# secondmind-labs/trieste

Hardware: NVIDIA H100
Metric: acquisition candidate-points/sec (EI on GPR N=4096 fp64) (higher is better)
Workload: dtype f64

## Files before the change

trieste_b200/csrc/kernels_f64.cuh:

```cuda
#pragma once
#include "common.cuh"
#include "../../include/trieste_b200.h"
#include "kernel_fn.cuh"
#include <cfloat>

namespace tb {

template <int KIND, int DP>
__global__ void __launch_bounds__(512)
kstar_panels_kernel(const double* __restrict__ Xs,
                    const double* __restrict__ alpha,
                    const double* __restrict__ Xc,
                    const double* __restrict__ inv_ls,
                    int N, int nkc, int D, int64_t M, int64_t cand0, double variance,
                    double mean_const, double* __restrict__ KsP, double* __restrict__ mean_out) {
  const int lane = threadIdx.x & 31, tj = threadIdx.x >> 5;
  const int tl = lane >> 2, kq = lane & 3;
  const int t_local = tj * 8 + tl;
  const int64_t t = cand0 + (int64_t)blockIdx.x * BT + t_local;
  const bool valid = t < M;

  double xc[DP];
#pragma unroll
  for (int d = 0; d < DP; ++d) xc[d] = (valid && d < D) ? Xc[t * D + d] * inv_ls[d] : 0.0;
// ... 379 lines not shown
}
__device__ __forceinline__ double gibbon_repulsion_value(double var, double noise, double uu, double w) {
  const double yvar = var + noise;
  return w * (0.5 * (log(yvar - uu) - log(yvar)));
}
__device__ __forceinline__ double gibbon_value(int acq, const double* __restrict__ samp, int ns, double mean, double var,
                                               double noise, double uu, double w) {
  if (acq == TB_ACQ_GIBBON_QUALITY) return gibbon_quality_value(samp, ns, mean, var, noise);
  const double rep = gibbon_repulsion_value(var, noise, uu, w);
  if (acq == TB_ACQ_GIBBON_REPULSION) return rep;
  return rep + gibbon_quality_value(samp, ns, mean, var, noise);
}

__device__ __forceinline__ void penalty_factor(int kind, double dist, double radius, double scale, double& f, double& w) {
  if (kind == TB_PEN_SOFT) {
    const double z = (dist - radius) / scale;
    f = ndtr_tfp(z);
    double lc, ratio;
    mes_terms(-z, lc, ratio);
    w = dist > 0.0 ? ratio / (scale * dist) : 0.0;
  } else {
    const double u = dist / (radius + scale);
    f = pow(pow(u, -5.0) + 1.0, -0.2);
    const double u5 = u * u * u * u * u;
    w = dist > 0.0 ? (1.0 / dist) / (dist * (1.0 + u5)) : 0.0;
  }
}

constexpr int PEN_TILE = 32;
constexpr int PEN_DMAX = 32;

struct TailPenalty {
  const double* xc = nullptr;
  const double* pend = nullptr;
  const double* radius = nullptr;
  const double* scale = nullptr;
  double* grad = nullptr;
  int P = 0, D = 0, kind = 0;
  const double* gib_uu = nullptr;
  double gib_w = 0.0;
};

__device__ __forceinline__ void block_best_store(double bv, int64_t bi, double* __restrict__ blk_best, int64_t* __restrict__ blk_idx) {
#pragma unroll
  for (int o = 16; o > 0; o >>= 1) {
    double v2 = __shfl_xor_sync(0xffffffffu, bv, o);
    int64_t i2 = __shfl_xor_sync(0xffffffffu, bi, o);
    best_merge(bv, bi, v2, i2);
  }
  __shared__ double sv[8];
  __shared__ int64_t si[8];
  if ((threadIdx.x & 31) == 0) {
    sv[threadIdx.x >> 5] = bv;
    si[threadIdx.x >> 5] = bi;
  }
  __syncthreads();
  if (threadIdx.x == 0) {
    for (int w = 1; w < (int)(blockDim.x >> 5); ++w) best_merge(bv, bi, sv[w], si[w]);
    blk_best[blockIdx.x] = bv;
    blk_idx[blockIdx.x] = bi;
  }
}

__device__ __forceinline__ double chunk_raw_variance(const double* __restrict__ partial, int G, int64_t McPad, int64_t t,
                                                     double variance) {
  double ss = 0.0;
  for (int g = 0; g < G; ++g) ss += partial[(int64_t)g * McPad + t];
  return variance - ss;
}

template <bool PEN>
__global__ void __launch_bounds__(256)
tail_kernel(const double* __restrict__ partial, int G, int64_t McPad, const double* __restrict__ mean,
            int64_t Mc, int64_t idx0, double variance, int acq, double param, double aux,
            const double* __restrict__ samp, int nsamp, double* __restrict__ out_vals, double* __restrict__ out_mean, double* __restrict__ out_var,
            double* __restrict__ blk_best, int64_t* __restrict__ blk_idx, const int64_t* __restrict__ idx_map, const TailPenalty pen) {
  const int64_t t = (int64_t)blockIdx.x * blockDim.x + threadIdx.x;
  double bv = -INFINITY;
  int64_t bi = INT64_MAX;
  double vb = 0.0;
  if (t < Mc) {
    double var = fmax(chunk_raw_variance(partial, G, McPad, t, variance), 1e-12);
    double mu = mean[t];
    if (out_mean) out_mean[t] = mu;
    if (out_var) out_var[t] = var;
    if (acq >= 0) {
      double v = (acq == TB_ACQ_MES) ? mes_value(samp, nsamp, mu, var)
                 : (acq >= TB_ACQ_GIBBON_QUALITY)
                     ? gibbon_value(acq, samp, nsamp, mu, var, aux, pen.gib_uu ? pen.gib_uu[t] : 0.0, pen.gib_w)
                     : acq_value(acq, param, aux, mu, var);
      if (PEN) {
        vb = v;
      } else {
        if (out_vals) out_vals[t] = v;
        if (v == v) { bv = v; bi = idx_map ? idx_map[t] : idx0 + t; }
      }
    }
  }
  if (PEN) {
    __shared__ double sp[PEN_TILE * PEN_DMAX], sr[PEN_TILE], sc[PEN_TILE];
    const bool live = t < Mc && acq >= 0;
    const int D = pen.D;
    double x[PEN_DMAX], g[PEN_DMAX];
#pragma unroll
    for (int d = 0; d < PEN_DMAX; ++d) {
      x[d] = (live && d < D) ? pen.xc[t * D + d] : 0.0;
      g[d] = 0.0;
    }
    double prod = 1.0;
    for (int j0 = 0; j0 < pen.P; j0 += PEN_TILE) {
      const int nj = min(PEN_TILE, pen.P - j0);
      __syncthreads();
      for (int i = threadIdx.x; i < nj * D; i += blockDim.x) sp[i] = pen.pend[(int64_t)j0 * D + i];
      if (threadIdx.x < nj) {
        sr[threadIdx.x] = pen.radius[j0 + threadIdx.x];
        sc[threadIdx.x] = pen.scale[j0 + threadIdx.x];
      }
      __syncthreads();
      if (!live) continue;
      for (int j = 0; j < nj; ++j) {
        double r2 = 0.0;
#pragma unroll
        for (int d = 0; d < PEN_DMAX; ++d)
          if (d < D) {
            const double df = x[d] - sp[j * D + d];
            r2 = fma(df, df, r2);
          }
        double f, w;
        penalty_factor(pen.kind, sqrt(r2), sr[j], sc[j], f, w);
        prod *= f;
        if (pen.grad) {
#pragma unroll
          for (int d = 0; d < PEN_DMAX; ++d)
            if (d < D) g[d] = fma(w, x[d] - sp[j * D + d], g[d]);
        }
      }
    }
    if (live) {
      const double v = vb < 0.0 ? NAN : vb * prod;
      if (pen.grad) {
        double* gr = pen.grad + t * D;
#pragma unroll
        for (int d = 0; d < PEN_DMAX; ++d)
          if (d < D) gr[d] = fma(prod, gr[d], prod == 0.0 ? 0.0 : vb * (prod * g[d]));
      }
      if (out_vals) out_vals[t] = v;
      if (v == v) { bv = v; bi = idx_map ? idx_map[t] : idx0 + t; }
    }
  }
  if (blk_best == nullptr) return;
  block_best_store(bv, bi, blk_best, blk_idx);
}

__global__ void __launch_bounds__(256)
argmax_fold_kernel(const double* __restrict__ blk_best, const int64_t* __restrict__ blk_idx, int nblk,
                   double* __restrict__ run_best, int64_t* __restrict__ run_idx) {
  double bv = -INFINITY;
  int64_t bi = INT64_MAX;
  for (int i = threadIdx.x; i < nblk; i += blockDim.x) best_merge(bv, bi, blk_best[i], blk_idx[i]);
#pragma unroll
  for (int o = 16; o > 0; o >>= 1) {
    double v2 = __shfl_xor_sync(0xffffffffu, bv, o);
    int64_t i2 = __shfl_xor_sync(0xffffffffu, bi, o);
    best_merge(bv, bi, v2, i2);
  }
  __shared__ double sv[8];
  __shared__ int64_t si[8];
  if ((threadIdx.x & 31) == 0) {
    sv[threadIdx.x >> 5] = bv;
    si[threadIdx.x >> 5] = bi;
  }
  __syncthreads();
  if (threadIdx.x == 0) {
    for (int w = 1; w < 8; ++w) best_merge(bv, bi, sv[w], si[w]);
    double rv = *run_best;
    int64_t ri = *run_idx;
    best_merge(rv, ri, bv, bi);
    *run_best = rv;
    *run_idx = ri;
  }
}

__device__ __forceinline__ double screen_threshold(int acq, double tau, double var_ub) {
  const double m = acq == TB_ACQ_EI ? fma(0x1p-20, fabs(tau), 0x1p-36 * sqrt(var_ub)) : 0x1p-20 * fmax(1.0, fabs(tau));
  return tau - m;
}

}
```

trieste_b200/csrc/prescreen.cuh:

```cuda
#pragma once
#include <cuda_fp16.h>
#include "kernels_f64.cuh"

namespace tb {
namespace pre {

constexpr int KS = 64;
constexpr int KH = 32;
constexpr int TH = 256;
template <int DP> struct Cpt { static constexpr int value = DP <= 12 ? 4 : DP <= 20 ? 2 : 1; };
template <int DP> struct Row { static constexpr int W = ((DP + 3 + 3) / 4) * 4; };

__host__ __device__ constexpr int tc_nk(int dp) { return (3 * dp + 2 + 15) / 16; }
__host__ __device__ constexpr int tc_mt(int dp) { return tc_nk(dp) <= 2 ? 4 : tc_nk(dp) <= 4 ? 2 : 1; }
__host__ __device__ constexpr int tc_slices(int dp) { return tc_nk(dp) <= 2 ? 16 : 8; }
__host__ __device__ constexpr int tc_slice_bytes(int dp) { return 256 * tc_nk(dp) + 32; }
__host__ __device__ constexpr int tc_cands(int dp) { return 16 * tc_mt(dp) * (TH / 32); }

struct Bound {
  double rel;
  double lin;
  double lin_max;
  double abs;
  double safety;
// ... 143 lines not shown
  asm("mma.sync.aligned.m16n8k16.row.col.f32.f16.f16.f32 {%0,%1,%2,%3}, {%4,%5,%6,%7}, {%8,%9}, {%0,%1,%2,%3};"
      : "+f"(c[0]), "+f"(c[1]), "+f"(c[2]), "+f"(c[3])
      : "r"(a[0]), "r"(a[1]), "r"(a[2]), "r"(a[3]), "r"(b0), "r"(b1));
}

template <int KIND, int DP>
__global__ void __launch_bounds__(TH, 2)
tc_mean_bounds_kernel(const unsigned char* __restrict__ cols, int nsl, int npos_sl, const double* __restrict__ Xc,
                      const double* __restrict__ inv_ls, const double* __restrict__ centre, int D, int64_t M,
                      const __grid_constant__ Bound b, int acq, double param, double var_ub, double* __restrict__ out0,
                      double* __restrict__ out1, double* __restrict__ blk_best, int64_t* __restrict__ blk_idx) {
  constexpr int NK = tc_nk(DP), K = 16 * NK, MT = tc_mt(DP), SL = tc_slices(DP), SLB = tc_slice_bytes(DP);
  constexpr int CB = tc_cands(DP), STB = SL * SLB;
  constexpr int CAND_BYTES = CB * (2 * K + 4), SMEM = CAND_BYTES > 2 * STB ? CAND_BYTES : 2 * STB;
  static_assert(KIND != TB_MATERN12 && STB % 16 == 0 && SMEM <= 48 * 1024, "tc_mean_bounds_kernel geometry");
  __shared__ __align__(16) unsigned char sm[SMEM];
  const int64_t c0 = (int64_t)blockIdx.x * CB;
  {
    __half* sa = reinterpret_cast<__half*>(sm);
    float* sx2 = reinterpret_cast<float*>(sm + CB * 2 * K);
    for (int c = threadIdx.x; c < CB; c += TH) {
      const int64_t t = c0 + c;
      __half* row = sa + c * K;
      float x2 = 0.0f;
#pragma unroll
      for (int d = 0; d < DP; ++d) {
        const float x = (t < M && d < D) ? (float)((Xc[t * D + d] * inv_ls[d] - centre[d]) * b.pre) : 0.0f;
        x2 = fmaf(x, x, x2);
        const __half hi = __float2half_rn(x);
        row[d] = row[2 * DP + d] = hi;
        row[DP + d] = __float2half_rn(x - __half2float(hi));
      }
      row[3 * DP] = row[3 * DP + 1] = __float2half_rn(1.0f);
#pragma unroll
      for (int k = 3 * DP + 2; k < K; ++k) row[k] = __float2half_rn(0.0f);
      sx2[c] = x2;
    }
  }
  __syncthreads();
  const int warp = threadIdx.x >> 5, lane = threadIdx.x & 31, g = lane >> 2, tg = lane & 3;
  uint32_t af[MT][NK][4];
  float cx[MT][2];
#pragma unroll
  for (int m = 0; m < MT; ++m) {
    const int r = (warp * MT + m) * 16 + g;
    const __half* sa = reinterpret_cast<const __half*>(sm);
#pragma unroll
    for (int kk = 0; kk < NK; ++kk) {
      const __half* p = sa + r * K + kk * 16 + 2 * tg;
      af[m][kk][0] = *reinterpret_cast<const uint32_t*>(p);
      af[m][kk][1] = *reinterpret_cast<const uint32_t*>(p + 8 * K);
      af[m][kk][2] = *reinterpret_cast<const uint32_t*>(p + 8);
      af[m][kk][3] = *reinterpret_cast<const uint32_t*>(p + 8 * K + 8);
    }
    const float* sx2 = reinterpret_cast<const float*>(sm + CB * 2 * K);
    cx[m][0] = sx2[r];
    cx[m][1] = sx2[r + 8];
  }
  __syncthreads();

  auto stage_load = [&](int kc, int buf) {
    const unsigned char* src = cols + (int64_t)kc * STB;
#pragma unroll
    for (int i = 0; i < (STB / 16 + TH - 1) / TH; ++i) {
      const int e = i * TH + (int)threadIdx.x;
      if (e < STB / 16) asm volatile("cp.async.cg.shared.global [%0], [%1], 16;" ::"r"(smem_u32(sm + buf * STB + 16 * e)), "l"(src + 16 * e) : "memory");
    }
    asm volatile("cp.async.commit_group;" ::: "memory");
  };
  auto slice = [&](const unsigned char* sp, float (&acc)[MT][2]) {
    uint32_t bf[NK][2];
    if constexpr (NK % 2 == 0) {
#pragma unroll
      for (int kk = 0; kk < NK; kk += 2) {
        const uint4 v = reinterpret_cast<const uint4*>(sp)[(lane * NK + kk) / 2];
        bf[kk][0] = v.x, bf[kk][1] = v.y, bf[kk + 1][0] = v.z, bf[kk + 1][1] = v.w;
      }
    } else {
#pragma unroll
      for (int kk = 0; kk < NK; ++kk) {
        const uint2 v = reinterpret_cast<const uint2*>(sp)[lane * NK + kk];
        bf[kk][0] = v.x, bf[kk][1] = v.y;
      }
    }
    const float2 w = reinterpret_cast<const float2*>(sp + 256 * NK)[tg];
#pragma unroll
    for (int m = 0; m < MT; ++m) {
      float c[4] = {cx[m][0], cx[m][0], cx[m][1], cx[m][1]};
#pragma unroll
      for (int kk = 0; kk < NK; ++kk) mma_f16(c, af[m][kk], bf[kk][0], bf[kk][1]);
#pragma unroll
      for (int i = 0; i < 4; ++i) {
        acc[m][i >> 1] = fmaf(i & 1 ? w.y : w.x, kfun<KIND>(c[i]), acc[m][i >> 1]);
      }
    }
  };

  double pd[MT][2], qd[MT][2];
#pragma unroll
  for (int m = 0; m < MT; ++m) pd[m][0] = pd[m][1] = qd[m][0] = qd[m][1] = 0.0;
  const int nst = (nsl + SL - 1) / SL;
  stage_load(0, 0);
  for (int kc = 0; kc < nst; ++kc) {
    const int buf = kc & 1;
    if (kc + 1 < nst) {
      stage_load(kc + 1, buf ^ 1);
      asm volatile("cp.async.wait_group 1;" ::: "memory");
    } else {
      asm volatile("cp.async.wait_group 0;" ::: "memory");
    }
    __syncthreads();
    const unsigned char* st = sm + buf * STB;
    const int s0 = kc * SL, pe = min(SL, nsl - s0), bnd = min(max(npos_sl - s0, 0), pe);
    auto run = [&](int sa, int sb, double (&dd)[MT][2]) {
      float acc[MT][2];
#pragma unroll
      for (int m = 0; m < MT; ++m) acc[m][0] = acc[m][1] = 0.0f;
#pragma unroll 1
      for (int s = sa; s < sb; ++s) slice(st + s * SLB, acc);
#pragma unroll
      for (int m = 0; m < MT; ++m) dd[m][0] += (double)acc[m][0], dd[m][1] += (double)acc[m][1];
    };
    run(0, bnd, pd);
    run(bnd, pe, qd);
    __syncthreads();
  }
  double bv = -INFINITY;
  int64_t bi = INT64_MAX;
#pragma unroll
  for (int m = 0; m < MT; ++m)
#pragma unroll
    for (int h = 0; h < 2; ++h) {
      pd[m][h] += __shfl_xor_sync(0xffffffffu, pd[m][h], 1);
      qd[m][h] += __shfl_xor_sync(0xffffffffu, qd[m][h], 1);
      pd[m][h] += __shfl_xor_sync(0xffffffffu, pd[m][h], 2);
      qd[m][h] += __shfl_xor_sync(0xffffffffu, qd[m][h], 2);
      const int64_t t = c0 + (warp * MT + m) * 16 + g + 8 * h;
      if ((2 * m + h) % 4 != tg || t >= M) continue;
      const double x2 = (double)cx[m][h];
      const double lg = x2 < 0x1p28 ? b.lin * (x2 + b.x2max) : NAN;
      bound_out(b, t, lg, pd[m][h] - qd[m][h], pd[m][h] + qd[m][h], acq, param, var_ub, out0, out1, bv, bi);
    }
  if (acq >= 0) block_best_store(bv, bi, blk_best, blk_idx);
}

__global__ void probe_kernel(const double* __restrict__ Xc, int D, const int64_t* __restrict__ probe, double* __restrict__ xsel,
                             int64_t* __restrict__ isel) {
  int64_t p = *probe;
  if (p == INT64_MAX) p = 0;
  for (int d = threadIdx.x; d < D; d += blockDim.x) xsel[d] = Xc[p * D + d];
  if (threadIdx.x == 0) isel[0] = p;
}

__global__ void __launch_bounds__(256)
compact_kernel(const double* __restrict__ Xc, const double* __restrict__ ub, int64_t M, int64_t split, int D, double var_ub,
               int acq, const double* __restrict__ run_best, int64_t cap, unsigned long long* __restrict__ count,
               double* __restrict__ xsel, int64_t* __restrict__ isel) {
  const int64_t t = (int64_t)blockIdx.x * blockDim.x + threadIdx.x;
  const double thr = screen_threshold(acq, *run_best, var_ub);
  const bool keep = t < M && !(ub[t] < thr);
  const bool back = t >= split;
  const unsigned ball = __ballot_sync(0xffffffffu, keep);
  if (ball == 0u) return;
  const int lane = threadIdx.x & 31;
  const unsigned bb = __ballot_sync(0xffffffffu, keep && back), bf = ball & ~bb;
  unsigned long long base_f = 0, base_b = 0;
  if (lane == 0) {
    if (bf) base_f = atomicAdd(&count[0], (unsigned long long)__popc(bf));
    if (bb) base_b = atomicAdd(&count[1], (unsigned long long)__popc(bb));
  }
  base_f = __shfl_sync(0xffffffffu, base_f, 0);
  base_b = __shfl_sync(0xffffffffu, base_b, 0);
  if (!keep) return;
  const unsigned below = (1u << lane) - 1u;
  const int64_t r = back ? (int64_t)(base_b + (unsigned long long)__popc(bb & below)) : (int64_t)(base_f + (unsigned long long)__popc(bf & below));
  if (r >= cap) return;
  const int64_t pos = back ? cap - 1 - r : r;
  for (int d = 0; d < D; ++d) xsel[pos * D + d] = Xc[t * D + d];
  isel[pos] = t;
}

}
}
```

trieste_b200/csrc/tb_api.cu:

```cuda
#include "gp_handle.cuh"
#include "kernels_extra.cuh"
#include "prescreen.cuh"
#include "batch_ei.cuh"
#include "ehvi.cuh"
#include "int8_engines.h"
#include <chrono>
#include "factor.cuh"
#include "lbfgs.cuh"

using namespace tb;
namespace tb {
int kernels_init();
}

namespace tb {

__global__ void scale_inputs_kernel(const double* __restrict__ X, const double* __restrict__ inv_ls,
                                    int64_t N, int D, int DP, int64_t rows, double* __restrict__ Xs) {
  int64_t i = (int64_t)blockIdx.x * blockDim.x + threadIdx.x;
  if (i >= rows * DP) return;
  int64_t k = i / DP;
  int d = (int)(i % DP);
  Xs[i] = (k < N && d < D) ? X[k * D + d] * inv_ls[d] : 0.0;
}
// ... 978 lines not shown
                         + 4.01 * std::ldexp(1.0, -22)
                         + 1.01 * rd * std::ldexp(1.0, -25)
                         + pre::tc_nk(DP) * 2.01 * 24 * std::ldexp(1.0, -23);
    const double abs_q = 1.01 * rd * std::ldexp(1.0, -24) + std::ldexp(1.0, -25);
    const double lin_tc = cq * lin_q + l64;
    bool f16_ok = false;
    if (1.01 * lin_tc * (box2 + 1.01 * x2max) <= 0.5 * lin_max) {
      tc = prescreen_tc_columns(h, N, DP, W, &gp->pre_nsl, &gp->pre_npos_sl, &f16_ok);
      gp->pre_tc = f16_ok;
    }
    if (gp->pre_tc) {
      terms = 8.0 * gp->pre_nsl;
      lin = lin_tc;
      rel += cq * abs_q;
    }
  } else {
    lin = LN2 * u;
  }
  gp->pre_rel = 1.01 * rel;
  gp->pre_lin = 1.01 * lin;
  gp->pre_lin_max = lin_max;
  gp->pre_abs = 1.01 * (asum * (2700.0 * std::ldexp(1.0, -126) + kappa * tail) + 2.0 * terms * std::ldexp(1.0, -149));
  gp->pre_scale = pre;
  gp->pre_x2max = 1.01 * x2max;
  const size_t bytes = gp->pre_tc ? tc.size() : sizeof(float) * h.size();
  TB_TRY(gp->dPreRows.reserve(bytes));
  TB_TRY(gp->dPreCentre.reserve(sizeof(double) * DP));
  TB_CUDA(cudaMemcpyAsync(gp->dPreRows.p, gp->pre_tc ? (const void*)tc.data() : (const void*)h.data(), bytes, cudaMemcpyHostToDevice, st));
  TB_CUDA(cudaMemcpyAsync(gp->dPreCentre.p, centre.data(), sizeof(double) * DP, cudaMemcpyHostToDevice, st));
  TB_CUDA(cudaStreamSynchronize(st));
  gp->pre_gen = gp->cache_gen;
  return 0;
}

static int prescreen_blocks(const tb_gp* gp, int64_t M) {
  const int DP = gp->DP;
  const int64_t per = gp->pre_tc ? pre::tc_cands(DP) : (int64_t)pre::TH * (DP <= 12 ? 4 : DP <= 20 ? 2 : 1);
  return (int)((M + per - 1) / per);
}

static int launch_mean_bounds(tb_gp* gp, cudaStream_t st, const double* Xc, int64_t M, int acq, double param, double var_ub,
                              double* out0, double* out1, double* blk_best, int64_t* blk_idx) {
  TB_TRY(prescreen_ensure(gp));
  pre::Bound b;
  b.rel = gp->pre_rel;
  b.lin = gp->pre_lin;
  b.lin_max = gp->pre_lin_max;
  b.abs = gp->pre_abs;
  b.safety = 4.0;
  b.x2max = gp->pre_x2max;
  b.mean_const = gp->mean_const;
  b.pre = gp->pre_scale;
  const int D = gp->D;
  const double* il = gp->dInvLs.as<double>();
  const double* cen = gp->dPreCentre.as<double>();
  const unsigned blocks = (unsigned)prescreen_blocks(gp, M);
  with_kind_dp(gp->kernel, gp->DP, [&](auto K, auto P) {
    constexpr int KIND = decltype(K)::value, DP = decltype(P)::value;
    if (!gp->pre_tc) {
      const int nst = (int)((gp->N + pre::KS - 1) / pre::KS);
      pre::mean_bounds_kernel<KIND, DP><<<blocks, pre::TH, 0, st>>>(gp->dPreRows.as<float>(), nst, Xc, il, cen, D, M, b, acq, param,
                                                                    var_ub, out0, out1, blk_best, blk_idx);
    } else if constexpr (KIND != TB_MATERN12) {
      pre::tc_mean_bounds_kernel<KIND, DP><<<blocks, pre::TH, 0, st>>>(gp->dPreRows.as<unsigned char>(), gp->pre_nsl, gp->pre_npos_sl,
                                                                       Xc, il, cen, D, M, b, acq, param, var_ub, out0, out1, blk_best,
                                                                       blk_idx);
    }
  });
  TB_LAUNCHED();
  TB_CUDA(cudaGetLastError());
  return 0;
}

enum class Engine {
  F64,
  OZ21,
  OZ15,
};

static int select_engine(tb_gp* gp, bool need_v, Engine* eng) {
  if (!(gp->engine == 1 && gp->N <= 16384)) {
    if (need_v) TB_TRY(ensure_upper_panels(gp));
    *eng = Engine::F64;
    return 0;
  }
  if (need_v) TB_TRY(ensure_kinv_dense(gp));
  bool single_pass;
  TB_TRY(int8_select(gp, need_v, &single_pass));
  *eng = single_pass ? Engine::OZ15 : Engine::OZ21;
  return 0;
}

static int eng_tile_width(const tb_gp* gp, Engine e) { return e == Engine::F64 ? BT : int8_tile_width(gp, e == Engine::OZ15); }
static size_t eng_tile_bytes(const tb_gp* gp, Engine e) {
  return e == Engine::F64 ? (size_t)gp->nkc * PANEL * sizeof(double) : int8_tile_bytes(gp, e == Engine::OZ15);
}

static int eng_groups(const tb_gp* gp, Engine e, int tiles) {
  const int fill = (2 * NUM_SMS + tiles - 1) / tiles;
  if (e == Engine::F64) return tiles >= NUM_SMS ? 1 : std::max(1, std::min(fill, gp->NB));
  return std::max(std::max(1, (gp->NB + 3) / 4), std::min(gp->NB, fill));
}

static int eng_kstar(tb_gp* gp, Engine e, const double* xc, int64_t mc, int tiles, const KSplit* split = nullptr, bool wide = false) {
  double* mean = gp->sMean.as<double>();
  if (e == Engine::F64) return launch_kstar(gp, xc, mc, tiles, gp->sKs.as<double>(), mean);
  return int8_kstar(gp, e == Engine::OZ15, xc, mc, tiles, gp->sKs.as<int8_t>(), mean, split, wide);
}

static int eng_variance(tb_gp* gp, Engine e, int tiles, int G, int64_t McPad, bool packed_a, int kper = 0) {
  cudaStream_t st = gp->stream;
  double* partial = gp->sPartial.as<double>();
  if (e != Engine::F64) return int8_variance(gp, e == Engine::OZ15, gp->sKs.as<int8_t>(), tiles, G, McPad, partial, kper);
  if (packed_a)
    trigemm_kernel<false, EPI_SUMSQ_PACKED><<<dim3(tiles, G), TG_THREADS, TG_SMEM, st>>>(
        gp->dLinvP.as<double>(), gp->sKs.as<double>(), gp->NB, gp->nkc, G, McPad, partial, gp->sA.as<double>(), nullptr, 0);
  else
    trigemm_kernel<false, EPI_SUMSQ><<<dim3(tiles, G), TG_THREADS, TG_SMEM, st>>>(
        gp->dLinvP.as<double>(), gp->sKs.as<double>(), gp->NB, gp->nkc, G, McPad, partial, nullptr, nullptr, 0);
  TB_LAUNCHED();
  TB_CUDA(cudaGetLastError());
  return 0;
}

static int eng_store_a(tb_gp* gp, Engine e, int tiles, int64_t McPad, double* out) {
  const int64_t lda = (int64_t)gp->NB * BM;
  const int G = eng_groups(gp, e, tiles);
  if (e != Engine::F64) return int8_store(gp, e == Engine::OZ15, false, gp->sKs.as<int8_t>(), tiles, G, McPad, out, lda);
  trigemm_kernel<false, EPI_PLAIN><<<dim3(tiles, G), TG_THREADS, TG_SMEM, gp->stream>>>(gp->dLinvP.as<double>(), gp->sKs.as<double>(),
                                                                                        gp->NB, gp->nkc, G, McPad, nullptr, nullptr, out, lda);
  TB_LAUNCHED();
  TB_CUDA(cudaGetLastError());
  return 0;
}

static int eng_store_v(tb_gp* gp, Engine e, int tiles, int64_t McPad) {
  const int64_t ldv = (int64_t)gp->NB * BM;
  double* V = gp->sV.as<double>();
  if (e == Engine::OZ21) {
    const int G = std::max(1, std::min(gp->NB, std::max((gp->NB + 7) / 8, (2 * NUM_SMS + tiles - 1) / tiles)));
    return int8_store(gp, false, true, gp->sKs.as<int8_t>(), tiles, G, McPad, V, ldv);
  }
  const int G = eng_groups(gp, e, tiles);
  if (e == Engine::OZ15) return int8_store(gp, true, true, gp->sKs.as<int8_t>(), tiles, G, McPad, V, ldv);
  trigemm_kernel<true, EPI_PLAIN><<<dim3(tiles, G), TG_THREADS, TG_SMEM, gp->stream>>>(gp->dLinvTP.as<double>(), gp->sA.as<double>(), gp->NB,
                                                                                       gp->NB * (BM / BK), G, McPad, nullptr, nullptr, V, ldv);
  TB_LAUNCHED();
  TB_CUDA(cudaGetLastError());
  return 0;
}


static int argmax_reset(tb_gp* gp) {
  const double init_v = -INFINITY;
  const int64_t init_i = INT64_MAX;
  TB_CUDA(cudaMemcpyAsync(gp->sRun.p, &init_v, 8, cudaMemcpyHostToDevice, gp->stream));
  TB_CUDA(cudaMemcpyAsync((char*)gp->sRun.p + 8, &init_i, 8, cudaMemcpyHostToDevice, gp->stream));
  return 0;
}
static int argmax_begin(tb_gp* gp, int64_t chunk_cap) {
  const int tail_blocks_cap = (int)((chunk_cap + 255) / 256);
  TB_TRY(gp->sRun.reserve(16));
  TB_TRY(gp->sBlkBest.reserve(sizeof(double) * tail_blocks_cap));
  TB_TRY(gp->sBlkIdx.reserve(sizeof(int64_t) * tail_blocks_cap));
  return argmax_reset(gp);
}
static int argmax_fold(tb_gp* gp, int64_t n) {
  argmax_fold_kernel<<<1, 256, 0, gp->stream>>>(gp->sBlkBest.as<double>(), gp->sBlkIdx.as<int64_t>(), (int)((n + 255) / 256),
                                                gp->sRun.as<double>(), reinterpret_cast<int64_t*>((char*)gp->sRun.p + 8));
  TB_LAUNCHED();
  return 0;
}
static int argmax_end(tb_gp* gp, EvalRequest& rq) {
  TB_CUDA(cudaMemcpyAsync(&rq.best_value, gp->sRun.p, 8, cudaMemcpyDeviceToHost, gp->stream));
  TB_CUDA(cudaMemcpyAsync(&rq.best_index, (char*)gp->sRun.p + 8, 8, cudaMemcpyDeviceToHost, gp->stream));
  return 0;
}

template <class F>
static int profiled_gemm(tb_gp* gp, double flops, F&& launch) {
  if (!gp->profile) return launch();
  cudaEvent_t e0 = nullptr, e1 = nullptr;
  TB_CUDA(cudaEventCreate(&e0));
  TB_CUDA(cudaEventCreate(&e1));
  TB_CUDA(cudaEventRecord(e0, gp->stream));
  TB_TRY(launch());
  TB_CUDA(cudaEventRecord(e1, gp->stream));
  gp->prof_events.emplace_back(e0, e1);
  gp->prof_event_flops.push_back(flops);
  return 0;
}
static int profile_fold(tb_gp* gp) {
  for (size_t i = 0; i < gp->prof_events.size(); ++i) {
    float ms = 0.f;
    TB_CUDA(cudaEventElapsedTime(&ms, gp->prof_events[i].first, gp->prof_events[i].second));
    gp->prof_ms += ms;
    gp->prof_flops += gp->prof_event_flops[i];
    gp->prof_launches += 1;
    cudaEventDestroy(gp->prof_events[i].first);
    cudaEventDestroy(gp->prof_events[i].second);
  }
  gp->prof_events.clear();
  gp->prof_event_flops.clear();
  return 0;
}

struct EvalOut {
  double *vals = nullptr, *mean = nullptr, *var = nullptr, *grad = nullptr;
};

static int member_step(tb_gp* gp, Engine e, const double* xc, int64_t n, int Gfix, bool grad, int* G, int64_t* McPad,
                       const KSplit* split = nullptr, bool spread = false) {
  const int nt = eng_tile_width(gp, e);
  const int tiles = (int)((n + nt - 1) / nt);
  *G = Gfix ? Gfix : eng_groups(gp, e, tiles);
  *McPad = (int64_t)tiles * nt;
  const int kper = spread && e != Engine::F64 ? int8_split_kper(gp, e == Engine::OZ15, tiles, *G) : 0;
  TB_TRY(eng_kstar(gp, e, xc, n, tiles, split, kper > 0));
  TB_TRY(profiled_gemm(gp, (double)*McPad * (double)gp->N * (double)gp->N,
                       [&] { return eng_variance(gp, e, tiles, *G, *McPad, grad, kper); }));
  return grad ? eng_store_v(gp, e, tiles, *McPad) : 0;
}

static int eval_chunk(tb_gp* gp, const EvalRequest& rq, Engine e, const double* xc, int64_t n, int64_t c0, int Gfix, const EvalOut& o,
                      const int64_t* idx_map = nullptr, const KSplit* split = nullptr) {
  cudaStream_t st = gp->stream;
  const double* partial = gp->sPartial.as<double>();
  const double* mean = gp->sMean.as<double>();
  int G;
  int64_t McPad;
  TB_TRY(member_step(gp, e, xc, n, Gfix, o.grad != nullptr, &G, &McPad, split, idx_map != nullptr));
  if (o.grad) {
    TB_TRY(launch_partials(gp, st, rq.acq, rq.param, partial, G, McPad, mean, xc, n));
    TB_TRY(launch_grad(gp, xc, n, o.grad));
  }
  TB_TRY(launch_tail(gp, st, rq, partial, G, McPad, mean, n, c0, o.vals, o.mean, o.var, xc, o.grad, idx_map));
  return rq.want_argmax ? argmax_fold(gp, n) : 0;
}

static int argmax_screened(tb_gp* gp, const EvalRequest& rq, Engine e, int64_t chunk_cap, int G, bool* done) {
  *done = false;
  cudaStream_t st = gp->stream;
  const int D = gp->D, nt = eng_tile_width(gp, e);
  const int64_t M = rq.M;
  const int64_t cap = std::max<int64_t>(1, M / 4);
  TB_TRY(prescreen_ensure(gp));
  const int sblocks = (int)((M + 255) / 256), bblocks = prescreen_blocks(gp, M);
  TB_TRY(gp->sScrUb.reserve(sizeof(double) * (size_t)M));
  TB_TRY(gp->sScrX.reserve(sizeof(double) * (size_t)cap * D));
  TB_TRY(gp->sScrIdx.reserve(sizeof(int64_t) * (size_t)cap));
  TB_TRY(gp->sScrBlk.reserve(16 * (size_t)bblocks + 32));
  double* ub = gp->sScrUb.as<double>();
  double* xsel = gp->sScrX.as<double>();
  int64_t* isel = gp->sScrIdx.as<int64_t>();
  double* bb = gp->sScrBlk.as<double>();
  int64_t* bi = reinterpret_cast<int64_t*>(bb + bblocks);
  double* probe_v = reinterpret_cast<double*>(bi + bblocks);
  int64_t* probe_i = reinterpret_cast<int64_t*>(probe_v + 1);
  unsigned long long* count = reinterpret_cast<unsigned long long*>(probe_v + 2);
  const int64_t split = ((M - 1) / chunk_cap) * chunk_cap;
  const KSplit ks_full = int8_kstar_split(gp, e == Engine::OZ15, (int)(chunk_cap / nt)),
               ks_last = int8_kstar_split(gp, e == Engine::OZ15, (int)((M - split + nt - 1) / nt));
  const bool same_split = ks_full.ksplit == ks_last.ksplit && ks_full.kc_per == ks_last.kc_per;
  const double var_ub = std::fmax(gp->variance, 1e-12);
  const double init_v = -INFINITY;
  const int64_t init_i = INT64_MAX;
  TB_CUDA(cudaMemcpyAsync(probe_v, &init_v, 8, cudaMemcpyHostToDevice, st));
  TB_CUDA(cudaMemcpyAsync(probe_i, &init_i, 8, cudaMemcpyHostToDevice, st));
  TB_TRY(launch_mean_bounds(gp, st, rq.Xc, M, rq.acq, rq.param, var_ub, ub, nullptr, bb, bi));
  argmax_fold_kernel<<<1, 256, 0, st>>>(bb, bi, bblocks, probe_v, probe_i);
  TB_LAUNCHED();
  pre::probe_kernel<<<1, 32, 0, st>>>(rq.Xc, D, probe_i, xsel, isel);
  TB_LAUNCHED();
  bool probe_last = true;
  if (!same_split) {
    int64_t p = 0;
    TB_CUDA(cudaMemcpyAsync(&p, probe_i, 8, cudaMemcpyDeviceToHost, st));
    TB_CUDA(cudaStreamSynchronize(st));
    probe_last = (p == INT64_MAX ? 0 : p) >= split;
  }
  const EvalOut none;
  TB_TRY(eval_chunk(gp, rq, e, xsel, 1, 0, G, none, isel, probe_last ? &ks_last : &ks_full));
  TB_CUDA(cudaMemsetAsync(count, 0, 16, st));
  pre::compact_kernel<<<sblocks, 256, 0, st>>>(rq.Xc, ub, M, split, D, var_ub, rq.acq, gp->sRun.as<double>(), cap, count, xsel, isel);
  TB_LAUNCHED();
  unsigned long long n[2] = {0, 0};
  TB_CUDA(cudaMemcpyAsync(n, count, 16, cudaMemcpyDeviceToHost, st));
  TB_CUDA(cudaStreamSynchronize(st));
  TB_CUDA(cudaGetLastError());
  if (n[0] + n[1] > (unsigned long long)cap) return argmax_reset(gp);
  const int64_t nf = (int64_t)n[0], nb = (int64_t)n[1];
  for (int64_t s0 = 0; s0 < nf; s0 += chunk_cap)
    TB_TRY(eval_chunk(gp, rq, e, xsel + s0 * D, std::min<int64_t>(chunk_cap, nf - s0), 0, G, none, isel + s0, &ks_full));
  for (int64_t s0 = cap - nb; s0 < cap; s0 += chunk_cap)
    TB_TRY(eval_chunk(gp, rq, e, xsel + s0 * D, std::min<int64_t>(chunk_cap, cap - s0), 0, G, none, isel + s0, &ks_last));
  *done = true;
  return 0;
}

struct ChunkPlan {
  int64_t chunk_cap = 0;
  int G[EHVI_LMAX] = {};
};
static ChunkPlan plan_chunks(tb_gp* const* gps, const Engine* eng, int n, bool grad, int64_t M) {
  ChunkPlan p;
  const size_t budget = (size_t)1280 << 20;
  for (int l = 0; l < n; ++l) {
    const tb_gp* gp = gps[l];
    const Engine e = eng[l];
    const int nt = eng_tile_width(gp, e);
    int64_t max_tiles;
    if (e != Engine::F64 && !grad) {
      max_tiles = std::max<int64_t>(1, (int64_t)(budget / eng_tile_bytes(gp, e)));
      if (max_tiles >= 2 * NUM_SMS) max_tiles = (max_tiles / (2 * NUM_SMS)) * (2 * NUM_SMS);
      else if (max_tiles >= NUM_SMS) max_tiles = NUM_SMS;
      max_tiles = std::min<int64_t>(max_tiles, 8 * NUM_SMS);
    } else if (e == Engine::OZ15) {
      const size_t v_bytes = (size_t)nt * gp->NB * BM * sizeof(double);
      max_tiles = std::max<int64_t>(1, (int64_t)(budget / std::max(eng_tile_bytes(gp, e), v_bytes)));
      if (max_tiles >= NUM_SMS) max_tiles = (max_tiles / NUM_SMS) * NUM_SMS;
    } else {
      max_tiles = chunk_tiles(gp);
    }
    const int64_t cap = std::min<int64_t>(max_tiles * nt, ((M + nt - 1) / nt) * nt);
    p.chunk_cap = l == 0 ? cap : std::min(p.chunk_cap, cap);
  }
  for (int l = 0; l < n; ++l) {
    const int nt = eng_tile_width(gps[l], eng[l]);
    if (eng[l] != Engine::F64 && !grad) p.G[l] = eng_groups(gps[l], eng[l], (int)((p.chunk_cap + nt - 1) / nt));
  }
  return p;
}

static int reserve_chunk(tb_gp* gp, Engine e, bool grad, int64_t chunk_cap, int G) {
  const int nt = eng_tile_width(gp, e);
  const int64_t tiles_cap = (chunk_cap + nt - 1) / nt, pad_cap = tiles_cap * nt;
  TB_TRY(gp->sKs.reserve((size_t)tiles_cap * eng_tile_bytes(gp, e)));
  TB_TRY(gp->sPartial.reserve(sizeof(double) * (size_t)(G ? G : gp->NB) * pad_cap));
  TB_TRY(gp->sMean.reserve(sizeof(double) * pad_cap));
  if (grad) {
    if (e == Engine::F64) TB_TRY(gp->sA.reserve((size_t)tiles_cap * gp->NB * (BM / BK) * PANEL * sizeof(double)));
    TB_TRY(gp->sV.reserve((size_t)pad_cap * gp->NB * BM * sizeof(double)));
    TB_TRY(gp->sMisc.reserve(sizeof(double) * 2 * pad_cap));
  }
  return 0;
}

static int check_eval(const tb_gp* gp, const EvalRequest& rq) {
  TB_CHECK(gp->cache_valid, "posterior cache is not built: call tb_gp_update_posterior_cache first");
  TB_CHECK(rq.M >= 0, "negative candidate count");
  if (rq.want_argmax) TB_CHECK(rq.M > 0, "argmax over an empty candidate set");
  return 0;
}

static int run_eval(tb_gp* gp, EvalRequest& rq) {
  TB_CUDA(cudaSetDevice(gp->device));
  cudaStream_t st = gp->stream;
  const int D = gp->D;
  const bool grad = rq.out_grad != nullptr;
  if (rq.M == 0) return 0;
  if (grad) TB_CHECK(rq.acq >= 0, "gradients need an acquisition kind");
  Engine e;
  TB_TRY(select_engine(gp, grad, &e));
  const ChunkPlan cp = plan_chunks(&gp, &e, 1, grad, rq.M);
  const int64_t chunk_cap = cp.chunk_cap;
  const Staged<const double> xin(rq.Xc, D, gp->sXc, st);
  const Staged<double> vals(rq.out_vals, 1, gp->sVals, st), mean(rq.out_mean, 1, gp->sMean, st), var(rq.out_var, 1, gp->sVar, st),
      grads(rq.out_grad, D, gp->sGrad, st);
  TB_TRY(reserve_chunk(gp, e, grad, chunk_cap, cp.G[0]));
  TB_TRY(xin.reserve(chunk_cap));
  TB_TRY(vals.reserve(chunk_cap));
  TB_TRY(var.reserve(chunk_cap));
  TB_TRY(grads.reserve(chunk_cap));
  if (rq.want_argmax) TB_TRY(argmax_begin(gp, chunk_cap));

  bool screened = false;
  if (e != Engine::F64 && argmax_screen_wanted(rq, xin.dev)) TB_TRY(argmax_screened(gp, rq, e, chunk_cap, cp.G[0], &screened));
  const int64_t m_loop = screened ? 0 : rq.M;
  for (int64_t c0 = 0; c0 < m_loop; c0 += chunk_cap) {
    const int64_t mc = std::min<int64_t>(chunk_cap, rq.M - c0);
    const double* xc;
    TB_TRY(xin.in(c0, mc, &xc));
    EvalOut o;
    o.vals = vals.out(c0);
    o.mean = mean.host() ? nullptr : mean.out(c0);
    o.var = var.out(c0);
    o.grad = grads.out(c0);
    TB_TRY(eval_chunk(gp, rq, e, xc, mc, c0, cp.G[0], o));
    TB_TRY(grads.back(c0, mc));
    TB_TRY(vals.back(c0, mc));
    TB_TRY(mean.back(c0, mc));
    TB_TRY(var.back(c0, mc));
  }
  if (rq.want_argmax) TB_TRY(argmax_end(gp, rq));
  TB_CUDA(cudaStreamSynchronize(st));
  TB_CUDA(cudaGetLastError());
  return profile_fold(gp);
}

static int run_mean_grad(tb_gp* gp, const double* Xc, int64_t M, double* mean, double* grad) {
  if (M == 0) return 0;
  TB_CUDA(cudaSetDevice(gp->device));
  cudaStream_t st = gp->stream;
  const int D = gp->D;
  constexpr int64_t CHUNK = 65536;
  const int64_t cap = std::min(M, CHUNK);
  const Staged<const double> xin(Xc, D, gp->sXc, st);
  const Staged<double> means(mean, 1, gp->sMean, st), grads(grad, D, gp->sGrad, st);
  TB_TRY(xin.reserve(cap));
  TB_TRY(means.reserve(cap));
  TB_TRY(grads.reserve(cap));
  const double* Xs = gp->dXs.as<double>();
  const double* al = gp->dAlpha.as<double>();
  const double* il = gp->dInvLs.as<double>();
  for (int64_t c0 = 0; c0 < M; c0 += CHUNK) {
    const int64_t mc = std::min(CHUNK, M - c0);
    const double* xc;
    TB_TRY(xin.in(c0, mc, &xc));
    double* md = means.out(c0);
    double* gd = grads.out(c0);
    const unsigned blocks = (unsigned)((mc + 7) / 8);
    with_kind_dp(gp->kernel, gp->DP, [&](auto K, auto P) {
      mean_grad_kernel<decltype(K)::value, decltype(P)::value><<<blocks, 256, 0, st>>>(Xs, al, xc, il, (int)gp->N, D, mc, gp->variance,
                                                                                       gp->mean_const, md, gd);
    });
    TB_LAUNCHED();
    TB_CUDA(cudaGetLastError());
    TB_TRY(means.back(c0, mc));
    TB_TRY(grads.back(c0, mc));
  }
  TB_CUDA(cudaStreamSynchronize(st));
  TB_CUDA(cudaGetLastError());
  return 0;
}

static int ensure_gibbon(tb_gp* gp) {
  TB_CHECK(gp->cache_valid, "GIBBON repulsion: posterior cache is not built: call tb_gp_update_posterior_cache first");
  if (gp->gib_gen == gp->cache_gen) return 0;
  TB_CUDA(cudaSetDevice(gp->device));
  cudaStream_t st = gp->stream;
  const int m = gp->gibM, D = gp->D, DP = gp->DP;
  const int mp = ((m + GIB_TILE - 1) / GIB_TILE) * GIB_TILE;
  const int N = (int)gp->N;
  std::vector<double> ps((size_t)m * DP, 0.0);
  for (int j = 0; j < m; ++j)
// ... 1528 lines not shown
```

Baseline: 322.2 million.

## Speculatively evaluate first compacted tile before host sync; replace tiny H2D copies with kernels

In the screened argmax path, when both split configurations match, all survivors are compacted into the front region. One tile of them is padded with the probe point and evaluated on the GPU before the host reads the survivor count, so that work overlaps the device-to-host synchronisation round trip. The host loop then skips the already evaluated prefix. Pageable host-to-device memcpys that initialise the running best are replaced by a one-thread init kernel, and the two result readbacks are merged into a single 16-byte copy followed by an explicit sync. The speculative tile may do redundant work when few candidates survive, and it relies on cap being at least nt for the prefix skip to stay correct.

```diff
diff --git a/trieste_b200/csrc/kernels_f64.cuh b/trieste_b200/csrc/kernels_f64.cuh
--- a/trieste_b200/csrc/kernels_f64.cuh
+++ b/trieste_b200/csrc/kernels_f64.cuh
@@ -555,6 +555,11 @@
   block_best_store(bv, bi, blk_best, blk_idx);
 }
 
+__global__ void argmax_init_kernel(double* __restrict__ run_best, int64_t* __restrict__ run_idx) {
+  *run_best = -INFINITY;
+  *run_idx = INT64_MAX;
+}
+
 __global__ void __launch_bounds__(256)
 argmax_fold_kernel(const double* __restrict__ blk_best, const int64_t* __restrict__ blk_idx, int nblk,
                    double* __restrict__ run_best, int64_t* __restrict__ run_idx) {
diff --git a/trieste_b200/csrc/prescreen.cuh b/trieste_b200/csrc/prescreen.cuh
--- a/trieste_b200/csrc/prescreen.cuh
+++ b/trieste_b200/csrc/prescreen.cuh
@@ -319,6 +319,18 @@
   if (threadIdx.x == 0) isel[0] = p;
 }
 
+__global__ void pad_kernel(const double* __restrict__ Xc, int D, const int64_t* __restrict__ probe,
+                           const unsigned long long* __restrict__ count, int64_t cap, int64_t spec, double* __restrict__ xsel,
+                           int64_t* __restrict__ isel) {
+  int64_t p = *probe;
+  if (p == INT64_MAX) p = 0;
+  const int64_t n = (int64_t)min(*count, (unsigned long long)cap);
+  for (int64_t s = n + threadIdx.x; s < spec; s += blockDim.x) {
+    for (int d = 0; d < D; ++d) xsel[s * D + d] = Xc[p * D + d];
+    isel[s] = p;
+  }
+}
+
 __global__ void __launch_bounds__(256)
 compact_kernel(const double* __restrict__ Xc, const double* __restrict__ ub, int64_t M, int64_t split, int D, double var_ub,
                int acq, const double* __restrict__ run_best, int64_t cap, unsigned long long* __restrict__ count,
diff --git a/trieste_b200/csrc/tb_api.cu b/trieste_b200/csrc/tb_api.cu
--- a/trieste_b200/csrc/tb_api.cu
+++ b/trieste_b200/csrc/tb_api.cu
@@ -1154,10 +1154,8 @@
 
 
 static int argmax_reset(tb_gp* gp) {
-  const double init_v = -INFINITY;
-  const int64_t init_i = INT64_MAX;
-  TB_CUDA(cudaMemcpyAsync(gp->sRun.p, &init_v, 8, cudaMemcpyHostToDevice, gp->stream));
-  TB_CUDA(cudaMemcpyAsync((char*)gp->sRun.p + 8, &init_i, 8, cudaMemcpyHostToDevice, gp->stream));
+  argmax_init_kernel<<<1, 1, 0, gp->stream>>>(gp->sRun.as<double>(), reinterpret_cast<int64_t*>((char*)gp->sRun.p + 8));
+  TB_LAUNCHED();
   return 0;
 }
 static int argmax_begin(tb_gp* gp, int64_t chunk_cap) {
@@ -1174,8 +1172,15 @@
   return 0;
 }
 static int argmax_end(tb_gp* gp, EvalRequest& rq) {
-  TB_CUDA(cudaMemcpyAsync(&rq.best_value, gp->sRun.p, 8, cudaMemcpyDeviceToHost, gp->stream));
-  TB_CUDA(cudaMemcpyAsync(&rq.best_index, (char*)gp->sRun.p + 8, 8, cudaMemcpyDeviceToHost, gp->stream));
+  struct {
+    double v;
+    int64_t i;
+  } run;
+  static_assert(sizeof(run) == 16, "gp->sRun holds the best value, then its index");
+  TB_CUDA(cudaMemcpyAsync(&run, gp->sRun.p, 16, cudaMemcpyDeviceToHost, gp->stream));
+  TB_CUDA(cudaStreamSynchronize(gp->stream));
+  rq.best_value = run.v;
+  rq.best_index = run.i;
   return 0;
 }
 
@@ -1249,8 +1254,13 @@
   TB_TRY(prescreen_ensure(gp));
   const int sblocks = (int)((M + 255) / 256), bblocks = prescreen_blocks(gp, M);
   TB_TRY(gp->sScrUb.reserve(sizeof(double) * (size_t)M));
-  TB_TRY(gp->sScrX.reserve(sizeof(double) * (size_t)cap * D));
-  TB_TRY(gp->sScrIdx.reserve(sizeof(int64_t) * (size_t)cap));
+  const int64_t split = ((M - 1) / chunk_cap) * chunk_cap;
+  const KSplit ks_full = int8_kstar_split(gp, e == Engine::OZ15, (int)(chunk_cap / nt)),
+               ks_last = int8_kstar_split(gp, e == Engine::OZ15, (int)((M - split + nt - 1) / nt));
+  const bool same_split = ks_full.ksplit == ks_last.ksplit && ks_full.kc_per == ks_last.kc_per;
+  const int64_t spec = same_split ? nt : 0;
+  TB_TRY(gp->sScrX.reserve(sizeof(double) * (size_t)std::max(cap, spec) * D));
+  TB_TRY(gp->sScrIdx.reserve(sizeof(int64_t) * (size_t)std::max(cap, spec)));
   TB_TRY(gp->sScrBlk.reserve(16 * (size_t)bblocks + 32));
   double* ub = gp->sScrUb.as<double>();
   double* xsel = gp->sScrX.as<double>();
@@ -1260,15 +1270,9 @@
   double* probe_v = reinterpret_cast<double*>(bi + bblocks);
   int64_t* probe_i = reinterpret_cast<int64_t*>(probe_v + 1);
   unsigned long long* count = reinterpret_cast<unsigned long long*>(probe_v + 2);
-  const int64_t split = ((M - 1) / chunk_cap) * chunk_cap;
-  const KSplit ks_full = int8_kstar_split(gp, e == Engine::OZ15, (int)(chunk_cap / nt)),
-               ks_last = int8_kstar_split(gp, e == Engine::OZ15, (int)((M - split + nt - 1) / nt));
-  const bool same_split = ks_full.ksplit == ks_last.ksplit && ks_full.kc_per == ks_last.kc_per;
   const double var_ub = std::fmax(gp->variance, 1e-12);
-  const double init_v = -INFINITY;
-  const int64_t init_i = INT64_MAX;
-  TB_CUDA(cudaMemcpyAsync(probe_v, &init_v, 8, cudaMemcpyHostToDevice, st));
-  TB_CUDA(cudaMemcpyAsync(probe_i, &init_i, 8, cudaMemcpyHostToDevice, st));
+  argmax_init_kernel<<<1, 1, 0, st>>>(probe_v, probe_i);
+  TB_LAUNCHED();
   TB_TRY(launch_mean_bounds(gp, st, rq.Xc, M, rq.acq, rq.param, var_ub, ub, nullptr, bb, bi));
   argmax_fold_kernel<<<1, 256, 0, st>>>(bb, bi, bblocks, probe_v, probe_i);
   TB_LAUNCHED();
@@ -1284,15 +1288,21 @@
   const EvalOut none;
   TB_TRY(eval_chunk(gp, rq, e, xsel, 1, 0, G, none, isel, probe_last ? &ks_last : &ks_full));
   TB_CUDA(cudaMemsetAsync(count, 0, 16, st));
-  pre::compact_kernel<<<sblocks, 256, 0, st>>>(rq.Xc, ub, M, split, D, var_ub, rq.acq, gp->sRun.as<double>(), cap, count, xsel, isel);
-  TB_LAUNCHED();
+  pre::compact_kernel<<<sblocks, 256, 0, st>>>(rq.Xc, ub, M, spec ? M : split, D, var_ub, rq.acq, gp->sRun.as<double>(), cap, count,
+                                               xsel, isel);
+  TB_LAUNCHED();
+  if (spec) {
+    pre::pad_kernel<<<1, 256, 0, st>>>(rq.Xc, D, probe_i, count, cap, spec, xsel, isel);
+    TB_LAUNCHED();
+    TB_TRY(eval_chunk(gp, rq, e, xsel, spec, 0, G, none, isel, &ks_full));
+  }
   unsigned long long n[2] = {0, 0};
   TB_CUDA(cudaMemcpyAsync(n, count, 16, cudaMemcpyDeviceToHost, st));
   TB_CUDA(cudaStreamSynchronize(st));
   TB_CUDA(cudaGetLastError());
   if (n[0] + n[1] > (unsigned long long)cap) return argmax_reset(gp);
   const int64_t nf = (int64_t)n[0], nb = (int64_t)n[1];
-  for (int64_t s0 = 0; s0 < nf; s0 += chunk_cap)
+  for (int64_t s0 = spec; s0 < nf; s0 += chunk_cap)
     TB_TRY(eval_chunk(gp, rq, e, xsel + s0 * D, std::min<int64_t>(chunk_cap, nf - s0), 0, G, none, isel + s0, &ks_full));
   for (int64_t s0 = cap - nb; s0 < cap; s0 += chunk_cap)
     TB_TRY(eval_chunk(gp, rq, e, xsel + s0 * D, std::min<int64_t>(chunk_cap, cap - s0), 0, G, none, isel + s0, &ks_last));
```

Result: slower. 311.0 million, median of 6 (-3.5%).
